# yuguangnudt/VEC_VAD

Hardware: AMD Instinct MI355X
Metric: spatio-temporal cubes/sec (train step) (higher is better)
Workload: dtype f32

## Files before the change

### include/vecvad_hip.h

```cpp
#ifndef VECVAD_HIP_H
#define VECVAD_HIP_H

#include <stddef.h>
#include <stdint.h>

#ifdef __cplusplus
extern "C" {
#endif

typedef void* vv_stream;

enum vv_status {
  VV_OK = 0,
  VV_ERR_BAD_ARG = 1,
  VV_ERR_LAUNCH = 2,
  VV_ERR_UNSUPPORTED = 3
};

enum vv_in_mode {
  VV_IN_PLAIN = 0,
  VV_IN_ACT = 1,
  VV_IN_POOL = 2,
  VV_IN_CAT = 3,
  VV_IN_CUBE = 4,
// ... 113 lines not shown

int vv_bn_finalize(int32_t G, int32_t C, int32_t ntiles, int64_t count, int32_t train, float momentum, float eps,
                   const float* stats, int64_t stats_gstride, const float* gamma, const float* beta,
                   int64_t param_gstride, float* running_mean, float* running_var, int64_t buf_gstride,
                   float* a, float* b, float* mean, float* invstd, int64_t ab_gstride, vv_stream stream);

#define VV_BNBWD_DZ_BF16 1
#define VV_BNBWD_PARTIALS_PER_CUBE 2
#define VV_BNBWD_Y_BF16 8
#define VV_BNBWD_DA_BF16 4
#define VV_BNBWD_PARTIALS_PER_TILE 16
#define VV_BNBWD_PARTIALS_PER_CTILE 32
#define VV_BNBWD_PARTIALS_PER_TTILE 128
#define VV_BNBWD_PARTIALS_PER_TILE44 64
typedef struct vv_bnbwd_params {
  int32_t G, B, H, W, C;
  int32_t flags;
  const float* y; int64_t y_gstride;
  const float* a; const float* b; const float* mean; const float* invstd; int64_t ab_gstride;
  vv_view dA;
  const float* dpool; int64_t dpool_gstride;
  float* dz; int64_t dz_gstride;
  float* partial;
} vv_bnbwd_params;
int vv_bn_bwd_reduce(const vv_bnbwd_params* p, vv_stream stream);
int vv_bn_bwd_nblk(int32_t B, int32_t H, int32_t W, int32_t C);
int vv_bn_bwd_apply(const vv_bnbwd_params* p, const float* gamma, int64_t param_gstride, float* dgamma, float* dbeta,
                    int64_t grad_gstride, float* scratch , vv_stream stream);
#define VV_BNBWD_TAB_ROWS 7
int vv_bn_bwd_sums(const vv_bnbwd_params* p, const float* gamma, int64_t param_gstride, float* dgamma, float* dbeta,
                   int64_t grad_gstride, float* table, int64_t table_gstride, vv_stream stream);

typedef struct vv_outconv_params {
  int32_t G, B, HW, C;
  const float* y; int64_t y_gstride; const float* a; const float* b; int64_t ab_gstride;
  const float* w; const float* bias; int64_t param_gstride;
  const int32_t* oc;
  const float* tgt0; int32_t tgt0_cstride; int32_t pad0;
  const float* tgt1; int32_t tgt1_cstride; int32_t pad1;
  const int32_t* tgt_src;
  const int32_t* tgt_coff;
  float* out4;
  float* score;
  const float* gscale;
  float* dout4;
} vv_outconv_params;
// ... 138 lines not shown
```

### vec_vad_amd/_lib.py

```python
import ctypes as C
import os

import torch

HERE = os.path.dirname(os.path.abspath(__file__))
LIB_PATH = os.environ.get('VV_LIB_PATH') or os.path.join(HERE, 'csrc', 'libvecvad_hip.so')

c_i32, c_i64, c_f32, c_f64, c_vp = C.c_int32, C.c_int64, C.c_float, C.c_double, C.c_void_p

IN_PLAIN, IN_ACT, IN_POOL, IN_CAT, IN_CUBE, IN_BNBWD = 0, 1, 2, 3, 4, 5
BNBWD_TAB_ROWS = 7
CONV3, CONVT_FWD, CONVT_DGRAD = 0, 1, 2
CONV_BF16 = 1
CONV_SRC_BF16 = 2
PACK_BF16 = 4
BNBWD_DZ_BF16 = 1
BNBWD_PARTIALS_PER_CUBE = 2
BNBWD_DA_BF16 = 4
CONV_OUT_BF16 = 8
CONV_ALLSRC_BF16 = 16
CONV_RELU = 32
CONV_NO_GEMM16 = 64
CONV_NO_RING = 128
BNBWD_Y_BF16 = 8
# ... 29 lines not shown
                ('dy', View), ('partial', c_vp), ('partial_gstride', c_i64),
                ('dy_z', View), ('dy_bn', c_vp), ('dy_bn_gstride', c_i64)]


class PackEntry(C.Structure):
    _fields_ = [('src_off', c_i64), ('dst_off', c_i64), ('mode', c_i32), ('K', c_i32), ('KP', c_i32), ('N', c_i32)]


class ReduceEntry(C.Structure):
    _fields_ = [('kind', c_i32), ('Cin', c_i32), ('Cout', c_i32), ('NCO', c_i32), ('nslab', c_i32), ('block_start', c_i32),
                ('part_off', c_i64), ('grad_off', c_i64), ('grad_gstride', c_i64)]


class FoldEntry(C.Structure):
    _fields_ = [('w_off', c_i64), ('b_off', c_i64), ('g_off', c_i64), ('beta_off', c_i64), ('rm_off', c_i64), ('rv_off', c_i64),
                ('cout', c_i32), ('row', c_i32)]


class BnBwdParams(C.Structure):
    _fields_ = [('G', c_i32), ('B', c_i32), ('H', c_i32), ('W', c_i32), ('C', c_i32), ('flags', c_i32),
                ('y', c_vp), ('y_gstride', c_i64),
                ('a', c_vp), ('b', c_vp), ('mean', c_vp), ('invstd', c_vp), ('ab_gstride', c_i64),
                ('dA', View), ('dpool', c_vp), ('dpool_gstride', c_i64),
                ('dz', c_vp), ('dz_gstride', c_i64), ('partial', c_vp)]


class OutconvParams(C.Structure):
    _fields_ = [('G', c_i32), ('B', c_i32), ('HW', c_i32), ('C', c_i32),
                ('y', c_vp), ('y_gstride', c_i64), ('a', c_vp), ('b', c_vp), ('ab_gstride', c_i64),
                ('w', c_vp), ('bias', c_vp), ('param_gstride', c_i64), ('oc', c_vp),
                ('tgt0', c_vp), ('tgt0_cstride', c_i32), ('pad0', c_i32),
                ('tgt1', c_vp), ('tgt1_cstride', c_i32), ('pad1', c_i32),
                ('tgt_src', c_vp), ('tgt_coff', c_vp), ('out4', c_vp), ('score', c_vp), ('gscale', c_vp),
                ('dout4', c_vp)]


class Conv2dParams(C.Structure):
    _fields_ = [('kind', c_i32), ('R', c_i32), ('stride', c_i32), ('B', c_i32), ('H', c_i32), ('W', c_i32),
                ('Cin', c_i32), ('CinP', c_i32), ('Cout', c_i32), ('CoutP', c_i32), ('src', View), ('w', c_vp),
                ('bias', c_vp), ('slope', c_f32), ('pad0', c_i32), ('out', View)]


_SIGS = {
    'vv_conv2d_mfma': (c_i32, [C.POINTER(Conv2dParams), c_vp]),
    'vv_conv2d_wino': (c_i32, [c_vp, c_i32, c_i32, c_i64, c_vp, c_vp, c_f32, c_vp, c_i32, c_i32, c_i32, c_i32, c_i32, c_i32, c_i32, c_vp]),
    'vv_conv2d_splitk_finish': (c_i32, [c_vp, c_i32, c_i64, c_i32, c_i32, c_vp, c_f32, c_vp, c_i32, c_i32, c_vp]),
    'vv_pack_conv2d': (c_i32, [c_vp, c_vp, c_i32, c_i32, c_i32, c_i32, c_i32, c_i32, c_vp]),
# ... 123 lines not shown
```

### vec_vad_amd/bank.py

```python
import ctypes as C
import math
import os
from collections import OrderedDict
from types import SimpleNamespace

import torch

from . import _lib as L

RAW_C, OF_C = 3, 2
HW0 = 32


def _ceil(a, b):
    return (a + b - 1) // b * b


def _pick_ksplit(groups, ntiles, ncu=256, epilogue=1.5, max_wg=1024):
    best, best_cost = 1, None
    for ks in range(1, ntiles + 1):
        if groups * ks > max_wg and ks > 1:
            break
        rounds = -(-groups * ks // ncu)
        cost = rounds * (-(-ntiles // ks) + epilogue)
# ... 158 lines not shown
        def launch_set(name, default, words, names):
            v = os.environ.get(name, default).lower()
            if v.startswith('set:'):
                picked = frozenset(t for t in v[4:].split(',') if t)
                if not picked <= names:
                    raise ValueError('%s=%s: unknown entries %s' % (name, v, sorted(picked - names)))
                return picked
            if v not in words:
                raise ValueError('%s must be one of %s or set:..., got %r' % (name, ' / '.join(words), v))
            return '0' if v == 'off' else v

        self.precision = os.environ.get('VV_PRECISION', 'fp32').lower()
        if self.precision not in ('fp32', 'bf16'):
            raise ValueError("VV_PRECISION / [mi355x] precision must be 'fp32' or 'bf16', got %r" % self.precision)
        if self.nf != 32 and self.precision != 'fp32':
            raise L.VecVadHipError('mixed precision is implemented for features_root = 32 only')
        self.cflag = L.CONV_BF16 if self.precision == 'bf16' else 0
        self.dz16 = switch('VV_BF16_DZ') and bool(self.cflag)
        self.da16 = switch('VV_BF16_DA') and bool(self.cflag)
        self.y16 = switch('VV_BF16_Y') and self.dz16 and self.da16
        self.split_dcat = switch('VV_SPLIT_DCAT') and self.da16
        self.fflag = self.cflag | ((L.CONV_OUT_BF16 | L.CONV_ALLSRC_BF16) if self.y16 else 0)
        self.fuse_outconv = switch('VV_FUSE_OUTCONV')
        wino_env = switch('VV_WINOGRAD')
        self.wino = wino_env and not self.cflag
        self.wino_wgrad = switch('VV_WINOGRAD_WGRAD') and wino_env
        self.wgrad_flag = 256
        w44_words = ('0', 'off', '1', 'dgrad', 'all')
        w44_names = frozenset(['f%d' % i for i in range(nconv)] + ['d%d' % i for i in range(1, nconv)])
        self.w44_mode = launch_set('VV_WINO44', 'dgrad', w44_words, w44_names)
        self._w44_tables = {}
        self._w44_eval_used = set()
        self.w44_eval_mode = launch_set('VV_WINO44_EVAL', '1', w44_words, w44_names)
        self.fuse_bn_sums = switch('VV_FUSE_BN_SUMS')
        self.fuse_bn_sums_t = switch('VV_FUSE_BN_SUMS_T')
        fold = launch_set('VV_FUSE_BN_APPLY', '1', ('0', 'off', '1'), frozenset(str(i) for i in range(nconv)))
        self.fold_bn_apply = frozenset(int(t) for t in fold) if isinstance(fold, frozenset) else \
            frozenset() if fold == '0' else frozenset((0, 2, 4))
        self.group_reduce = switch('VV_GROUP_REDUCE')
        self.eval_fold = switch('VV_EVAL_FOLD') and not self.cflag

        self.params = torch.zeros(G, lay.U, device=d)
        self.bufs = torch.zeros(G, lay.UB, device=d)
        self.gb = [0, lay.p['c4.w'][0], lay.p['c8.w'][0], lay.U]
        self._gb_c = (C.c_int64 * len(self.gb))(*self.gb)
        self.grads = torch.zeros(G * lay.U, device=d)
# ... 218 lines not shown
                    ents[i] = L.PackEntry(lay.p[src][0], off, mode, K, KP, N)
                    mx = max(mx, KP * N)
                self._w44_tables[B] = (torch.frombuffer(bytearray(bytes(ents)), dtype=torch.uint8).to(self.device), len(keys), mx)
        return self._w44_tables[B]

    def _src_for(self, ws, l):
        lay, Ga = self.lay, self.Ga
        abg = lay.cmax
        if l.mode == L.IN_CUBE:
            return (L.IN_PLAIN, L.view(ws.erased, l.cinp, 0, ws.erased.stride(0)), None, None, L.NULL_VIEW, 0, None)
        if l.mode == L.IN_POOL:
            pb = ws.pooled[l.idx]
            return (L.IN_PLAIN, L.view(pb, l.cin, 0, pb.stride(0)), None, None, L.NULL_VIEW, 0, None)
        if l.mode == L.IN_ACT:
            s = lay.convs[l.src]
            y = ws.y[s.idx]
            return (L.IN_ACT, L.view(y, s.cout, 0, y.stride(0)), self._p(ws.ab[0, s.idx]), self._p(ws.ab[1, s.idx]), L.NULL_VIEW, 0, None)
        s = lay.convs[l.skip]
        y, t = ws.y[s.idx], ws.t[l.up]
        return (L.IN_CAT, L.view(y, s.cout, 0, y.stride(0)), self._p(ws.ab[0, s.idx]), self._p(ws.ab[1, s.idx]),
                L.view(t, t.shape[2], 0, t.stride(0)), s.cout, None)

    def _alloc_outconv_bwd(self, ws, B):
        if hasattr(ws, 'gA_last'):
            return
        lib, lay, Ga = self.lib, self.lay, self.Ga
        d = self.device
        f = lambda *shape: torch.empty(*shape, device=d, dtype=torch.float32)
        HWp = HW0 * HW0
        ws.gA_last = f(Ga, B * HWp, self.nf)
        nblk = [lib.vv_bn_bwd_nblk(B, l.H, l.H, l.cout) for l in lay.convs]
        ws.bnpart = f(Ga, max(max(n, lib.vv_wino_ntiles(B, l.H), lib.vv_conv_ntiles(B, l.H, l.H),
                                  lib.vv_conv_ntiles2(B, l.H, l.H, L.CONV3, self.fflag),
                                  lib.vv_convt_dgrad_ntiles(B, l.H, l.H, 0))
                              * 2 * l.cout for n, l in zip(nblk, lay.convs)))
        ws.ocpart = f(Ga, B, 4 * self.nf + 4)

    def backward_plan(self, ws, fused):
        if ws.bwd is None:
            ws.bwd = self._plan_backward(ws, ws.B)
        if not fused:
            return ws.bwd
        if ws.bwdq is None:
            q = _Plan()
            q.keep = ws.bwd.keep
            for c, m in zip(ws.bwd.calls, ws.bwd.meta):
                if c[2] != 'outconv_bwd':
                    q.calls.append(c)
                    q.meta.append(m)
            ws.bwdq = q
        return ws.bwdq

    def _plan_forward(self, ws, B, train, out4=True):
# ... 49 lines not shown
                              L.view(t, co, 0, t.stride(0)), None)
            P.keep.append(cp)
            P.add(lib.vv_conv_mfma, (C.byref(cp),), 'convT%d' % u)

        P.add(lib.vv_cube_erase, (Ga, B * HW0 * HW0, ws.cube.shape[2], lay.convs[0].cinp, ws.cube.data_ptr(),
                                  self._p(self.chmap, g0 * lay.convs[0].cinp), ws.erased.data_ptr(), ws.erased.stride(0),
                                  1 if self.y16 else 0), 'cube_erase')
        for l in lay.convs:
            if l.mode == L.IN_CAT:
                convT(l.up)
            if l.mode == L.IN_POOL:
                s = lay.convs[l.src]
                ys, pb = ws.y[s.idx], ws.pooled[l.idx]
                P.add(lib.vv_pool_act, (Ga, B, l.H, l.H, s.cout, ys.data_ptr(), ys.stride(0), self._p(ws.ab[0, s.idx]),
                                        self._p(ws.ab[1, s.idx]), abg, pb.data_ptr(), pb.stride(0), 1 if self.y16 else 0), 'pool%d' % l.idx)
            conv(l)
        last = lay.convs[-1]
        y = ws.y[last.idx]
        op = L.OutconvParams(Ga, B, HW0 * HW0, self.nf, y.data_ptr(), y.stride(0), self._p(ws.ab[0, last.idx]),
                             self._p(ws.ab[1, last.idx]), abg, pbase + 4 * lay.p['o.w'][0], pbase + 4 * lay.p['o.b'][0], U,
                             self._p(self.oc, g0), ws.cube.data_ptr(), ws.cube.shape[2], 1 if self.y16 else 0, ws.flow.data_ptr(),
                             ws.flow.shape[2], 0, self._p(self.tsrc, g0), self._p(self.tcoff, g0), ws.out4.data_ptr() if out4 else None,
                             ws.score.data_ptr(), ws.gscale.data_ptr() if train else None,
                             ws.dout4.data_ptr() if (train and not (self.fuse_outconv and not out4)) else None)
        P.keep.append(op)
        if train and self.fuse_outconv and not out4:
            P.fused_outconv = True
            P.add(lib.vv_outconv_fwdbwd, (C.byref(op), ws.gA_last.data_ptr(), ws.gA_last.stride(0), ws.ocpart.data_ptr(),
                                          self._p(ws.ab[2, last.idx]), self._p(ws.ab[3, last.idx]), ws.bnpart.data_ptr(),
                                          (1 if self.da16 else 0) | (2 if self.y16 else 0)), 'outconv')
        else:
            P.add(lib.vv_outconv_fwd, (C.byref(op),), 'outconv')
        return P

    def mark_dirty(self):
        self._state_ver += 1

    def prepare_eval(self):
        key = (self._state_ver, self.params._version, self.bufs._version, self.params.data_ptr())
        if self._eval_key == key:
            return
        lib, lay, G = self.lib, self.lay, self.G
        if self.params_eval is None:
            self.params_eval = torch.empty_like(self.params)
            self.packed_eval = torch.zeros_like(self.packed)
        st = self._stream()
        self.params_eval.copy_(self.params)
        L.check(lib.vv_fold_bn(self.fold_table.data_ptr(), len(lay.convs), G, self.params.data_ptr(), lay.U, self.bufs.data_ptr(),
                               lay.UB, 1e-5, self.params_eval.data_ptr(), lay.U, st), 'fold_bn')
        L.check(lib.vv_pack_weights(self.pack_table.data_ptr(), self.pack_n, G, self.params_eval.data_ptr(), lay.U,
                                    self.packed_eval.data_ptr(), lay.UP, self.pack_max, st), 'pack (eval)')
# ... 90 lines not shown

        def dcat_views(m):
            dcat = ws.D[m.idx]
            skipc = lay.convs[m.skip].cout
            if self.split_dcat and 2 * skipc == m.cin and skipc & (skipc - 1) == 0:
                plane = B * m.H * m.H * skipc * 2
                return (L.view(dcat, skipc, 0, dcat.stride(0)), L.view(dcat.data_ptr() + plane, skipc, 0, dcat.stride(0)), skipc)
            return (L.view(dcat, m.cin, 0, dcat.stride(0)), L.View(dcat.data_ptr(), dcat.stride(0), m.cin, skipc), 0)
        ws.DT = [f(Ga, B * H * H, ci) for (_, H, ci, co) in lay.convT]
        ws.dz2 = [f(Ga, B * HWp * nf), f(Ga, B * HWp * nf)]
        ws.dz = ws.dz2[0]
        ws.bnscr = f(Ga, 2 * lay.cmax)
        ws.bscr = f(Ga, (B * HWp + 1023) // 1024 * lay.cmax)
        ws.dstats = f(Ga, max(max(lib.vv_conv_ntiles2(B, l.H, l.H, L.CONV3, self.cflag), lib.vv_conv_ntiles(B, l.H, l.H),
                                  lib.vv_wino_ntiles(B, l.H)) * 2 * l.cin for l in lay.convs if l.mode == L.IN_CAT))

        t_of = {sidx: u for u, (sidx, _, _, _) in enumerate(lay.convT)}
        skip_of = {m.skip: m for m in lay.convs if m.mode == L.IN_CAT}
        pool_of = {m.src: m for m in lay.convs if m.mode == L.IN_POOL}
        act_of = {m.src: m for m in lay.convs if m.mode == L.IN_ACT}

        def dA_for(i):
            if i == last.idx:
                return L.view(ws.gA_last, nf, 0, ws.gA_last.stride(0)), None, 0
            if i in t_of:
                t = ws.DT[t_of[i]]
                return L.view(t, t.shape[2], 0, t.stride(0)), None, 0
            if i in skip_of:
                dp = ws.D[pool_of[i].idx] if i in pool_of else None
                return dcat_views(skip_of[i])[0], dp.data_ptr() if dp is not None else None, dp.stride(0) if dp is not None else 0
            dn = ws.D[i + 1]
            return L.view(dn, lay.convs[i + 1].cin, 0, dn.stride(0)), None, 0

        def wgrad(kind, H, cinp, cout, bf16_flags, wide):
            tiles = ((cinp + 31) // 32) * (cout // 32)
            nt = lib.vv_wgrad_ntiles(kind, B, H, H)
            ks = _pick_ksplit(Ga * tiles, nt, ncu=3 * self.ncu, max_wg=12 * self.ncu) if wide else \
                _pick_ksplit(Ga * tiles, nt, ncu=self.ncu, max_wg=4 * self.ncu)
            w = SimpleNamespace(bf16=False, ks=ks, kw=0)
            ntb, nblk, kw = C.c_int32(), C.c_int32(), C.c_int32()
            if self.cflag and lib.vv_wgrad_bf16_plan(kind | (bf16_flags << 8), B, H, H, cinp, cout,
                                                     C.byref(ntb), C.byref(nblk), C.byref(kw)):
                w = SimpleNamespace(bf16=True, ks=self._ks_bf16(Ga * nblk.value, ntb.value), kw=kw.value)
            w.nslab = w.ks * max(w.kw, 1)
            w.size = tiles * w.nslab * 9 * 1024
            return w
# ... 44 lines not shown
                return
            pending.append((kind, cin, cinp, cout, w, gptr, gstride))
            if not bucket_done:
                return
            ents = (L.ReduceEntry * len(pending))()
            start = 0
            for n, (kind, cin, cinp, cout, w, gptr, gstride) in enumerate(pending):
                ents[n] = L.ReduceEntry(kind, cin, cout, cout // 32, w.nslab, start, w.woff, (gptr - self.grads.data_ptr()) // 4, gstride)
                start += ((cinp + 31) // 32) * (cout // 32) * 36
            tab = torch.frombuffer(bytearray(bytes(ents)), dtype=torch.uint8).to(d)
            P.keep.append(tab)
            P.add(lib.vv_wgrad_reduce_grouped, (tab.data_ptr(), len(pending), start, Ga, ws.wpart.data_ptr(), wpg, self.grads.data_ptr()),
                  label, stream=1, **kw_)
            del pending[:]

        def bn_sums(cp, j):
            yj = ws.y[j]
            cp.bn_z, cp.bn_z_gstride = yj.data_ptr(), yj.stride(0)
            cp.bn_a, cp.bn_b = self._p(ws.ab[0, j]), self._p(ws.ab[1, j])
            cp.bn_mean, cp.bn_invstd = self._p(ws.ab[2, j]), self._p(ws.ab[3, j])
            cp.bn_gstride, cp.bn_partial = abg, ws.bnpart.data_ptr()

        y = ws.y[last.idx]
        P.add(lib.vv_outconv_bwd, (Ga, B, HWp, nf, ws.dout4.data_ptr(), y.data_ptr(), y.stride(0), self._p(ws.ab[0, last.idx]),
                                   self._p(ws.ab[1, last.idx]), abg, pbase + 4 * lay.p['o.w'][0], U, ws.gA_last.data_ptr(),
                                   ws.gA_last.stride(0), ws.ocpart.data_ptr(),
                                   self._p(ws.ab[2, last.idx]), self._p(ws.ab[3, last.idx]), ws.bnpart.data_ptr(),
                                   (1 if self.da16 else 0) | (2 if self.y16 else 0)), 'outconv_bwd')
        assert self._g('o.w')[1] == self._g('o.b')[1]
        P.add(lib.vv_outconv_bwd_reduce, (Ga, nf, B, ws.ocpart.data_ptr(), self._p(self.oc, g0), self._g('o.w')[0],
                                          self._g('o.b')[0], self._g('o.w')[1]), 'outconv_bwd_reduce')

        order = [l.idx for l in reversed(lay.convs)]

        def conv_bwd(l):
            i, r = l.idx, rec[l.idx]
            y = ws.y[i]
            pos = order.index(i)
            dzb = ws.dz2[pos % 2]
            reuse_wait = ('wdone%d' % order[pos - 2],) if pos >= 2 and not r.fold else ()
            bp = L.BnBwdParams(Ga, B, l.H, l.H, l.cout,
                               (L.BNBWD_DZ_BF16 if r.dz16 else 0) | r.partials | (L.BNBWD_DA_BF16 if self.da16 else 0) |
                               (L.BNBWD_Y_BF16 if self.y16 else 0), y.data_ptr(), y.stride(0), self._p(ws.ab[0, i]), self._p(ws.ab[1, i]),
                               self._p(ws.ab[2, i]), self._p(ws.ab[3, i]), abg, r.dA, r.dpool, r.dpg, dzb.data_ptr(), dzb.stride(0),
                               ws.bnpart.data_ptr())
            P.keep.append(bp)
            if not r.partials:
                P.add(lib.vv_bn_bwd_reduce, (C.byref(bp),), 'bn_bwd_reduce%d' % i, wait=reuse_wait)
            if r.fold:
                tab = ws.bntab[i]
                P.add(lib.vv_bn_bwd_sums, (C.byref(bp), pbase + 4 * lay.p['c%d.g' % i][0], U, self._g('c%d.g' % i)[0],
                                           self._g('c%d.beta' % i)[0], self._g('c%d.g' % i)[1], tab.data_ptr(), tab.stride(0)),
                      'bn_bwd_sum%d' % i, record='dy%d' % i)
            else:
                P.add(lib.vv_bn_bwd_apply, (C.byref(bp), pbase + 4 * lay.p['c%d.g' % i][0], U, self._g('c%d.g' % i)[0],
                                            self._g('c%d.beta' % i)[0], self._g('c%d.g' % i)[1], ws.bnscr.data_ptr()), 'bn_bwd_apply%d' % i,
                      record='dy%d' % i, wait=reuse_wait if r.partials else ())
            if i > 0:
                Dl = ws.D[i]
                fn, panel = r.dgrad[:2]
                cp = L.ConvParams(L.CONV3, L.IN_PLAIN, Ga, B, l.H, l.H, l.cout, l.cout, l.cin,
                                  L.View(dzb.data_ptr(), dzb.stride(0), l.cout, 0), None, None, 0, L.NULL_VIEW, 0, r.dflags, None,
                                  kbase + 4 * panel, UP, None, 0, L.view(Dl, l.cin, 0, Dl.stride(0)),
                                  ws.dstats.data_ptr() if l.mode == L.IN_CAT else None)
                if r.fold:
                    cp.in_mode, cp.src0, cp.src1 = L.IN_BNBWD, r.dA, L.view(y, l.cout, 0, y.stride(0))
                    cp.a, cp.ab_gstride = ws.bntab[i].data_ptr(), ws.bntab[i].stride(0)
                if l.mode == L.IN_CAT:
# ... 186 lines not shown
```

### vec_vad_amd/csrc/vv_common.h

```cpp
#pragma once
#include <hip/hip_runtime.h>
#include <stdint.h>
#include <type_traits>
#include "../../include/vecvad_hip.h"

typedef float v16f __attribute__((ext_vector_type(16)));
typedef float v4f __attribute__((ext_vector_type(4)));

#define VV_WG 256

template <int B, int E, typename F>
__device__ __forceinline__ void vv_static_for(F&& f) {
  if constexpr (B < E) {
    f(std::integral_constant<int, B>{});
    vv_static_for<B + 1, E>(f);
  }
}

#define VV_LAUNCH(...)                  \
  do {                                  \
    (void)hipGetLastError();            \
    hipLaunchKernelGGL(__VA_ARGS__);    \
  } while (0)

// ... 37 lines not shown
__device__ __forceinline__ VVBnBwd4 vv_bnbwd_consts(const float* tab, const int C, const int c) {
  VVBnBwd4 k;
  k.a = *reinterpret_cast<const float4*>(tab + c);
  k.b = *reinterpret_cast<const float4*>(tab + C + c);
  k.m = *reinterpret_cast<const float4*>(tab + 2 * C + c);
  k.i = *reinterpret_cast<const float4*>(tab + 3 * C + c);
  k.gk = *reinterpret_cast<const float4*>(tab + 4 * C + c);
  k.c1 = *reinterpret_cast<const float4*>(tab + 5 * C + c);
  k.c2 = *reinterpret_cast<const float4*>(tab + 6 * C + c);
  return k;
}
__device__ __forceinline__ float vv_bnbwd1(float d, const float y, const float a, const float b, const float m, const float i,
                                           const float gk, const float c1, const float c2) {
  const float z = fmaf(a, y, b);
  d = z > 0.f ? d : 0.f;
  const float xh = (y - m) * i;
  return gk * (d - c1 - xh * c2);
}
__device__ __forceinline__ float4 vv_bnbwd4(const float4 d, const float4 y, const VVBnBwd4& k) {
  return make_float4(vv_bnbwd1(d.x, y.x, k.a.x, k.b.x, k.m.x, k.i.x, k.gk.x, k.c1.x, k.c2.x),
                     vv_bnbwd1(d.y, y.y, k.a.y, k.b.y, k.m.y, k.i.y, k.gk.y, k.c1.y, k.c2.y),
                     vv_bnbwd1(d.z, y.z, k.a.z, k.b.z, k.m.z, k.i.z, k.gk.z, k.c1.z, k.c2.z),
                     vv_bnbwd1(d.w, y.w, k.a.w, k.b.w, k.m.w, k.i.w, k.gk.w, k.c1.w, k.c2.w));
}
__device__ __forceinline__ float4 vv_max4(float4 p, float4 q) {
  p.x = fmaxf(p.x, q.x); p.y = fmaxf(p.y, q.y); p.z = fmaxf(p.z, q.z); p.w = fmaxf(p.w, q.w);
  return p;
}

typedef __bf16 v8bf __attribute__((ext_vector_type(8)));
typedef __bf16 v2bf __attribute__((ext_vector_type(2)));
typedef float v2f __attribute__((ext_vector_type(2)));
__device__ __forceinline__ v2f vv_pk_lo_pm_hi(const v2f x, const v2f y) {
  v2f r;
  asm("v_pk_add_f32 %0, %1, %2 op_sel:[0,1] op_sel_hi:[0,1] neg_hi:[0,1]" : "=v"(r) : "v"(x), "v"(y));
  return r;
}

template <int LPP>
__device__ __forceinline__ float vv_group_sum(float d) {
  static_assert(LPP == 8 || LPP == 16, "8 or 16 lanes per group");
  auto dpp = [](const float v, const auto CTRL) -> float {
    return __builtin_bit_cast(float, __builtin_amdgcn_update_dpp(0, __builtin_bit_cast(int, v), decltype(CTRL)::value, 0xF, 0xF, false));
  };
  d += dpp(d, std::integral_constant<int, 0xB1>{});
  d += dpp(d, std::integral_constant<int, 0x4E>{});
// ... 416 lines not shown
```

### vec_vad_amd/csrc/vv_elem.hip

```cpp
#include "vv_common.h"

namespace {

__global__ void __launch_bounds__(VV_WG)
pack_weights_kernel(const vv_pack_entry* __restrict__ table, const float* __restrict__ params,
                    const int64_t params_gstride, float* __restrict__ packed, const int64_t packed_gstride) {
  __shared__ float tile[8 * 32 * 9 + 8];
  const vv_pack_entry e = table[blockIdx.y];
  const int g = blockIdx.z;
  const float* src = params + (int64_t)g * params_gstride + e.src_off;
  float* dst = packed + (int64_t)g * packed_gstride + e.dst_off;
  const bool b16 = (e.mode & 4) != 0;
  const int m = e.mode & 3;
  const bool kmajor = m == 1 || m == 2;
  const bool flip = m == 1;
  const int NB = e.N >> 5, KB = e.KP >> 3;
  const int tid = threadIdx.x;
  for (int blk = blockIdx.x; blk < KB * NB; blk += gridDim.x) {
    const int kb = blk / NB, nb = blk % NB;
    const int k0 = kb * 8, n0 = nb * 32;
    __syncthreads();
    for (int i = tid; i < 8 * 32 * 9; i += VV_WG) {
      int64_t si;
      bool ok;
// ... 72 lines not shown
  double mu, var;
  if (train) {
    double s1 = 0.0, s2 = 0.0;
#pragma unroll
    for (int k = 0; k < VV_NP; ++k) { s1 += sh[0][k][cl]; s2 += sh[1][k][cl]; }
    mu = s1 / count;
    var = s2 / count - mu * mu;
    if (var < 0.0) var = 0.0;
    const double unb = count > 1.0 ? var * count / (count - 1.0) : var;
    *rm = (float)((1.0 - (double)momentum) * (double)*rm + (double)momentum * mu);
    *rv = (float)((1.0 - (double)momentum) * (double)*rv + (double)momentum * unb);
  } else {
    mu = (double)*rm;
    var = (double)*rv;
  }
  const double is = 1.0 / sqrt(var + (double)eps);
  const int64_t o = (int64_t)g * ab_gstride + c;
  a[o] = (float)((double)gm * is);
  b[o] = (float)((double)bt - mu * (double)gm * is);
  mean[o] = (float)mu;
  invstd[o] = (float)is;
}

template <bool POOL, int PASS>
__global__ void __launch_bounds__(VV_WG)
bn_bwd_reduce_kernel(const vv_bnbwd_params p, const int nblk, const int bp, const float* __restrict__ gamma,
                     const int64_t param_gstride, const float* __restrict__ scratch) {
  __shared__ float sh[2][VV_WG * 4];
  const int g = blockIdx.y, blk = blockIdx.x;
  const int C = p.C, Q4 = C >> 2, PL = VV_WG / Q4;
  const int q = threadIdx.x % Q4, pl = threadIdx.x / Q4;
  const int c = q * 4;
  const int64_t M = (int64_t)p.B * p.H * p.W;
  const float* __restrict__ y = p.y + (int64_t)g * p.y_gstride;
  float* __restrict__ dz = p.dz + (int64_t)g * p.dz_gstride;
  const float* __restrict__ dA = p.dA.ptr + (int64_t)g * p.dA.gstride + p.dA.coff;
  const int dcs = p.dA.cstride;
  const bool da16 = (p.flags & VV_BNBWD_DA_BF16) != 0;
  const unsigned short* __restrict__ dAh = reinterpret_cast<const unsigned short*>(p.dA.ptr + (int64_t)g * p.dA.gstride) + p.dA.coff;
  auto ldA = [&](const int64_t pix) -> float4 {
    if (da16) return vv_unpack_bf16x4(*reinterpret_cast<const uint2*>(dAh + pix * dcs + c));
    return *reinterpret_cast<const float4*>(dA + pix * dcs + c);
  };
  const int64_t abo = (int64_t)g * p.ab_gstride + c;
  const float4 a4 = *reinterpret_cast<const float4*>(p.a + abo), b4 = *reinterpret_cast<const float4*>(p.b + abo);
  const float4 m4 = *reinterpret_cast<const float4*>(p.mean + abo), i4 = *reinterpret_cast<const float4*>(p.invstd + abo);
  float4 s1 = make_float4(0, 0, 0, 0), s2 = make_float4(0, 0, 0, 0);
  VVBnBwd4 kc;
  if constexpr (PASS == 1) {
    const float4 gm = *reinterpret_cast<const float4*>(gamma + (int64_t)g * param_gstride + c);
    kc.a = a4; kc.b = b4; kc.m = m4; kc.i = i4;
    kc.gk = make_float4(gm.x * i4.x, gm.y * i4.y, gm.z * i4.z, gm.w * i4.w);
    kc.c1 = *reinterpret_cast<const float4*>(scratch + (int64_t)g * 2 * C + c);
    kc.c2 = *reinterpret_cast<const float4*>(scratch + (int64_t)g * 2 * C + C + c);
  }

  const bool y16 = (p.flags & VV_BNBWD_Y_BF16) != 0;
  auto ldY = [&](const int64_t pix) -> float4 {
    if (y16) return vv_unpack_bf16x4(*reinterpret_cast<const uint2*>(reinterpret_cast<const unsigned short*>(y) + pix * C + c));
    return *reinterpret_cast<const float4*>(y + pix * C + c);
  };
  auto one = [&](const int64_t pix, float4 d, const float4 yv) {
    if constexpr (PASS == 0) {
// ... 337 lines not shown
  const float4 a4 = *reinterpret_cast<const float4*>(a + abo), b4 = *reinterpret_cast<const float4*>(b + abo);
  float4 wv[4];
#pragma unroll
  for (int co = 0; co < 4; ++co) wv[co] = *reinterpret_cast<const float4*>(w + (int64_t)g * param_gstride + co * C + c);
  const float* __restrict__ yg = y + (int64_t)g * y_gstride;
  float* __restrict__ dAg = dA + (int64_t)g * dA_gstride;
  const int64_t MB = (int64_t)B * HW;
  float4 dw[4];
  float db[4] = {0, 0, 0, 0};
#pragma unroll
  for (int co = 0; co < 4; ++co) dw[co] = make_float4(0, 0, 0, 0);
  float4 m4 = make_float4(0, 0, 0, 0), i4 = m4, s1 = m4, s2 = m4;
  if (bnpart) { m4 = *reinterpret_cast<const float4*>(mean + abo); i4 = *reinterpret_cast<const float4*>(invstd + abo); }
  auto ldd = [&](const int i) -> float4 { return *reinterpret_cast<const float4*>(dout4 + ((int64_t)g * MB + (int64_t)cube * HW + i) * 4); };
  auto ldy = [&](const int i) -> float4 {
    const int64_t pix = (int64_t)cube * HW + i;
    return (dA_bf16 & 2) ? vv_unpack_bf16x4(*reinterpret_cast<const uint2*>(reinterpret_cast<const unsigned short*>(yg) + pix * C + c))
                         : *reinterpret_cast<const float4*>(yg + pix * C + c);
  };
  auto body = [&](const int i, const float4 d, const float4 yv) {
    const int64_t pix = (int64_t)cube * HW + i;
    const float4 v = vv_act4(yv, a4, b4);
    const float dd[4] = {d.x, d.y, d.z, d.w};
    float4 o = make_float4(0, 0, 0, 0);
#pragma unroll
    for (int co = 0; co < 4; ++co) {
      o.x = fmaf(dd[co], wv[co].x, o.x); o.y = fmaf(dd[co], wv[co].y, o.y);
      o.z = fmaf(dd[co], wv[co].z, o.z); o.w = fmaf(dd[co], wv[co].w, o.w);
      dw[co].x = fmaf(dd[co], v.x, dw[co].x); dw[co].y = fmaf(dd[co], v.y, dw[co].y);
      dw[co].z = fmaf(dd[co], v.z, dw[co].z); dw[co].w = fmaf(dd[co], v.w, dw[co].w);
      db[co] += dd[co];
    }
    if (dA_bf16 & 1) {
      const uint2 h = vv_pack_bf16x4(o);
      *reinterpret_cast<uint2*>(reinterpret_cast<unsigned short*>(dAg) + pix * C + c) = h;
      o = vv_unpack_bf16x4(h);
    } else {
      *reinterpret_cast<float4*>(dAg + pix * C + c) = o;
    }
    if (bnpart) {
      const float4 gq = make_float4(v.x > 0.f ? o.x : 0.f, v.y > 0.f ? o.y : 0.f, v.z > 0.f ? o.z : 0.f, v.w > 0.f ? o.w : 0.f);
      s1.x += gq.x; s1.y += gq.y; s1.z += gq.z; s1.w += gq.w;
      s2.x = fmaf(gq.x, (yv.x - m4.x) * i4.x, s2.x); s2.y = fmaf(gq.y, (yv.y - m4.y) * i4.y, s2.y);
      s2.z = fmaf(gq.z, (yv.z - m4.z) * i4.z, s2.z); s2.w = fmaf(gq.w, (yv.w - m4.w) * i4.w, s2.w);
    }
  };
  for (int i0 = pg; i0 < HW; i0 += 4 * NPG) {
    float4 d4[4], y4[4];
#pragma unroll
    for (int u = 0; u < 4; ++u)
      if (i0 + u * NPG < HW) { d4[u] = ldd(i0 + u * NPG); y4[u] = ldy(i0 + u * NPG); }
#pragma unroll
    for (int u = 0; u < 4; ++u)
      if (i0 + u * NPG < HW) body(i0 + u * NPG, d4[u], y4[u]);
  }
#pragma unroll
  for (int co = 0; co < 4; ++co) *reinterpret_cast<float4*>(&sh[pg][sub * 16 + co * 4]) = dw[co];
  if (sub == 0) {
#pragma unroll
    for (int co = 0; co < 4; ++co) sh[pg][LPP * 16 + co] = db[co];
// ... 348 lines not shown
    const int64_t pix = (int64_t)cube * p.HW + i;
    const float4 v = vv_act4(yv, a4, b4);
    float o[4];
#pragma unroll
    for (int co = 0; co < 4; ++co) {
      float d = v.x * wv[co].x;
      d = fmaf(v.y, wv[co].y, d); d = fmaf(v.z, wv[co].z, d); d = fmaf(v.w, wv[co].w, d);
      d = vv_group_sum<LPP>(d);
      o[co] = d + bias[co];
    }
    const float tv[4] = {tq.x, tq.y, tq.z, tq.w};
    float e[4] = {0, 0, 0, 0}, dd[4];
#pragma unroll
    for (int co = 0; co < 4; ++co) {
      if (co < oc) e[co] = o[co] - tv[co]; else o[co] = 0.f;
      dd[co] = gs * e[co];
    }
    if (sub == 0) {
#pragma unroll
      for (int co = 0; co < 4; ++co) if (co < oc) sse = fmaf(e[co], e[co], sse);
      if (p.out4) *reinterpret_cast<float4*>(p.out4 + ((int64_t)g * MB + pix) * 4) = make_float4(o[0], o[1], o[2], o[3]);
      if (p.dout4) *reinterpret_cast<float4*>(p.dout4 + ((int64_t)g * MB + pix) * 4) = make_float4(dd[0], dd[1], dd[2], dd[3]);
    }
    float4 q = make_float4(0, 0, 0, 0);
#pragma unroll
    for (int co = 0; co < 4; ++co) {
      q.x = fmaf(dd[co], wb[co].x, q.x); q.y = fmaf(dd[co], wb[co].y, q.y);
      q.z = fmaf(dd[co], wb[co].z, q.z); q.w = fmaf(dd[co], wb[co].w, q.w);
      dw[co].x = fmaf(dd[co], v.x, dw[co].x); dw[co].y = fmaf(dd[co], v.y, dw[co].y);
      dw[co].z = fmaf(dd[co], v.z, dw[co].z); dw[co].w = fmaf(dd[co], v.w, dw[co].w);
      db[co] += dd[co];
    }
    if (flags & 1) {
      const uint2 h = vv_pack_bf16x4(q);
      *reinterpret_cast<uint2*>(reinterpret_cast<unsigned short*>(dAg) + pix * C + c) = h;
      q = vv_unpack_bf16x4(h);
    } else {
      *reinterpret_cast<float4*>(dAg + pix * C + c) = q;
    }
    if (bnpart) {
      const float4 gq = make_float4(v.x > 0.f ? q.x : 0.f, v.y > 0.f ? q.y : 0.f, v.z > 0.f ? q.z : 0.f, v.w > 0.f ? q.w : 0.f);
      s1.x += gq.x; s1.y += gq.y; s1.z += gq.z; s1.w += gq.w;
      s2.x = fmaf(gq.x, (yv.x - m4.x) * i4.x, s2.x); s2.y = fmaf(gq.y, (yv.y - m4.y) * i4.y, s2.y);
      s2.z = fmaf(gq.z, (yv.z - m4.z) * i4.z, s2.z); s2.w = fmaf(gq.w, (yv.w - m4.w) * i4.w, s2.w);
    }
  };
  for (int i0 = pg; i0 < p.HW; i0 += 4 * NPG) {
    float4 yq4[4], tq4[4];
#pragma unroll
    for (int u = 0; u < 4; ++u)
      if (i0 + u * NPG < p.HW) { yq4[u] = ldy(i0 + u * NPG); tq4[u] = ldt(i0 + u * NPG); }
#pragma unroll
    for (int u = 0; u < 4; ++u)
      if (i0 + u * NPG < p.HW) body(i0 + u * NPG, yq4[u], tq4[u]);
  }
#pragma unroll
  for (int off = 32; off >= 1; off >>= 1) sse += __shfl_xor(sse, off);
  if ((tid & 63) == 0) red[tid >> 6] = sse;
#pragma unroll
  for (int co = 0; co < 4; ++co) *reinterpret_cast<float4*>(&sh[pg][sub * 16 + co * 4]) = dw[co];
// ... 336 lines not shown
  return (p->flags & VV_BNBWD_PARTIALS_PER_CUBE) ? p->B
         : (p->flags & VV_BNBWD_PARTIALS_PER_TILE) ? vv_wino_ntiles(p->B, p->H)
         : (p->flags & VV_BNBWD_PARTIALS_PER_TILE44) ? vv_wino44_ntiles(p->B, p->H)
         : (p->flags & VV_BNBWD_PARTIALS_PER_CTILE) ? vv_conv_ntiles(p->B, p->H, p->W)
         : (p->flags & VV_BNBWD_PARTIALS_PER_TTILE) ? vv_convt_dgrad_ntiles(p->B, p->H, p->W, 0) : bn_nblk_of(p);
}

extern "C" int vv_bn_bwd_sums(const vv_bnbwd_params* p, const float* gamma, int64_t param_gstride, float* dgamma, float* dbeta,
                              int64_t grad_gstride, float* table, int64_t table_gstride, vv_stream stream) {
  if (!p || !p->partial || !p->a || !p->b || !p->mean || !p->invstd || !gamma || !dgamma || !dbeta || !table) return VV_ERR_BAD_ARG;
  if (p->dpool || (p->flags & (VV_BNBWD_DZ_BF16 | VV_BNBWD_DA_BF16 | VV_BNBWD_Y_BF16))) return VV_ERR_UNSUPPORTED;
  if (table_gstride < (int64_t)VV_BNBWD_TAB_ROWS * p->C) return VV_ERR_BAD_ARG;
  const int nblk = bn_partial_rows(p);
  if (nblk <= 0) return VV_ERR_BAD_ARG;
  const int64_t M = (int64_t)p->B * p->H * p->W;
  VV_LAUNCH(bn_bwd_sum_kernel, dim3((p->C + 31) / 32, p->G), dim3(32 * VV_NP), 0, (hipStream_t)stream, p->C, nblk, (double)M,
            p->partial, dgamma, dbeta, grad_gstride, nullptr, *p, gamma, param_gstride, table, table_gstride);
  VV_CHECK_LAUNCH();
  return VV_OK;
}

extern "C" int vv_bn_bwd_apply(const vv_bnbwd_params* p, const float* gamma, int64_t param_gstride, float* dgamma,
                               float* dbeta, int64_t grad_gstride, float* scratch, vv_stream stream) {
  if (!p || !p->y || !p->dA.ptr || !p->dz || !p->partial || !gamma || !dgamma || !dbeta || !scratch) return VV_ERR_BAD_ARG;
  const int nblk = bn_partial_rows(p);
  if (nblk <= 0) return VV_ERR_BAD_ARG;
  const int nblk_apply = bn_nblk_of(p);
  const int64_t M = (int64_t)p->B * p->H * p->W;
  VV_LAUNCH(bn_bwd_sum_kernel, dim3((p->C + 31) / 32, p->G), dim3(32 * VV_NP), 0, (hipStream_t)stream, p->C, nblk, (double)M,
            p->partial, dgamma, dbeta, grad_gstride, scratch, *p, nullptr, 0, nullptr, 0);
  VV_CHECK_LAUNCH();
  if (bn_all16(p)) {
    if (p->dpool)
      VV_LAUNCH((bn_bwd16_kernel<true, 1>), dim3(nblk_apply, p->G), dim3(VV_WG), 0, (hipStream_t)stream, *p, nblk_apply, bn_bp_of(p), gamma, param_gstride, scratch);
    else
      VV_LAUNCH((bn_bwd16_kernel<false, 1>), dim3(nblk_apply, p->G), dim3(VV_WG), 0, (hipStream_t)stream, *p, nblk_apply, bn_bp_of(p), gamma, param_gstride, scratch);
  } else if (p->dpool)
    VV_LAUNCH((bn_bwd_reduce_kernel<true, 1>), dim3(nblk_apply, p->G), dim3(VV_WG), 0, (hipStream_t)stream, *p, nblk_apply, bn_bp_of(p), gamma, param_gstride, scratch);
  else
    VV_LAUNCH((bn_bwd_reduce_kernel<false, 1>), dim3(nblk_apply, p->G), dim3(VV_WG), 0, (hipStream_t)stream, *p, nblk_apply, bn_bp_of(p), gamma, param_gstride, scratch);
  VV_CHECK_LAUNCH();
  return VV_OK;
}

extern "C" int vv_outconv_fwd(const vv_outconv_params* p, vv_stream stream) {
  if (!p || !p->y || !p->a || !p->b || !p->w || !p->bias || !p->oc || !p->tgt_src || !p->tgt_coff || !p->score || !p->tgt0)
    return VV_ERR_BAD_ARG;
  if (p->pad0 & 1) return launch_outconv8<0>(*p, nullptr, nullptr, 0, nullptr, nullptr, nullptr, nullptr, true, false, (hipStream_t)stream);
  const int total = p->B * p->G, nper = (total + 7) / 8;
  if (p->C == 32) VV_LAUNCH(outconv_fwd_kernel<32>, dim3(nper * 8), dim3(VV_WG), 0, (hipStream_t)stream, *p, total, nper);
  else if (p->C == 64) VV_LAUNCH(outconv_fwd_kernel<64>, dim3(nper * 8), dim3(VV_WG), 0, (hipStream_t)stream, *p, total, nper);
  else return VV_ERR_UNSUPPORTED;
  VV_CHECK_LAUNCH();
  return VV_OK;
}

extern "C" int vv_outconv_fwdbwd(const vv_outconv_params* p, float* dA, int64_t dA_gstride, float* partial, const float* mean,
                                 const float* invstd, float* bnpart, int32_t flags, vv_stream stream) {
  if (!p || !p->y || !p->a || !p->b || !p->w || !p->bias || !p->oc || !p->tgt_src || !p->tgt_coff || !p->score || !p->tgt0 ||
      !p->gscale || !dA || !partial)
    return VV_ERR_BAD_ARG;
  if (bnpart && (!mean || !invstd)) return VV_ERR_BAD_ARG;
  if (((flags & 2) != 0) != ((p->pad0 & 1) != 0)) return VV_ERR_BAD_ARG;
  if (flags & 2) return launch_outconv8<2>(*p, nullptr, dA, dA_gstride, partial, mean, invstd, bnpart, true, (flags & 1) != 0, (hipStream_t)stream);
  const int total = p->B * p->G, nper = (total + 7) / 8;
  if (p->C == 32) VV_LAUNCH(outconv_fwdbwd_kernel<32>, dim3(nper * 8), dim3(VV_WG), 0, (hipStream_t)stream, *p, dA, dA_gstride, partial, mean, invstd, bnpart, flags, total, nper);
  else if (p->C == 64) VV_LAUNCH(outconv_fwdbwd_kernel<64>, dim3(nper * 8), dim3(VV_WG), 0, (hipStream_t)stream, *p, dA, dA_gstride, partial, mean, invstd, bnpart, flags, total, nper);
  else return VV_ERR_UNSUPPORTED;
  VV_CHECK_LAUNCH();
  return VV_OK;
}

extern "C" int vv_outconv_bwd_nblk(int32_t B, int32_t HW) { (void)HW; return B; }

extern "C" int vv_outconv_bwd(int32_t G, int32_t B, int32_t HW, int32_t C, const float* dout4, const float* y,
                              int64_t y_gstride, const float* a, const float* b, int64_t ab_gstride, const float* w,
                              int64_t param_gstride, float* dA, int64_t dA_gstride, float* partial,
                              const float* mean, const float* invstd, float* bnpart, int32_t dA_bf16, vv_stream stream) {
  if (!dout4 || !y || !a || !b || !w || !dA || !partial) return VV_ERR_BAD_ARG;
  if (bnpart && (!mean || !invstd)) return VV_ERR_BAD_ARG;
  if (dA_bf16 & 2) {
    vv_outconv_params p = {};
    p.G = G; p.B = B; p.HW = HW; p.C = C;
    p.y = y; p.y_gstride = y_gstride; p.a = a; p.b = b; p.ab_gstride = ab_gstride;
    p.w = w; p.param_gstride = param_gstride;
    return launch_outconv8<1>(p, dout4, dA, dA_gstride, partial, mean, invstd, bnpart, true, (dA_bf16 & 1) != 0, (hipStream_t)stream);
  }
  if (C == 32)
    VV_LAUNCH(outconv_bwd_kernel<32>, dim3(B, G), dim3(VV_WG), 0, (hipStream_t)stream, B, HW, C, dout4, y, y_gstride,
              a, b, ab_gstride, w, param_gstride, dA, dA_gstride, partial, mean, invstd, bnpart, dA_bf16);
  else if (C == 64)
    VV_LAUNCH(outconv_bwd_kernel<64>, dim3(B, G), dim3(VV_WG), 0, (hipStream_t)stream, B, HW, C, dout4, y, y_gstride,
              a, b, ab_gstride, w, param_gstride, dA, dA_gstride, partial, mean, invstd, bnpart, dA_bf16);
  else return VV_ERR_UNSUPPORTED;
  VV_CHECK_LAUNCH();
  return VV_OK;
}

extern "C" int vv_outconv_bwd_reduce(int32_t G, int32_t C, int32_t nblk, const float* partial, const int32_t* oc,
                                     float* dW, float* db, int64_t grad_gstride, vv_stream stream) {
  if (!partial || !oc || !dW || !db) return VV_ERR_BAD_ARG;
  if (C == 32) VV_LAUNCH(outconv_bwd_reduce_kernel<32>, dim3(G), dim3(1024), 0, (hipStream_t)stream, C, nblk, partial, oc, dW, db, grad_gstride);
// ... 222 lines not shown
```

Baseline: 29080.

## Recompute output-conv dA in BN backward apply instead of storing it

In fp32 mode by default, the outconv backward no longer writes the full-size dA tensor for the last layer. The BN backward apply kernel instead rebuilds dA on the fly from the 4-channel dout4 and the outconv weights. This removes a large write and read-back of B*HW*nf floats in exchange for a few extra FMAs per element. The dout4 buffer is now always written in the fused path, which adds a small store.

```diff
diff --git a/include/vecvad_hip.h b/include/vecvad_hip.h
--- a/include/vecvad_hip.h
+++ b/include/vecvad_hip.h
@@ -159,6 +159,7 @@
   const float* dpool; int64_t dpool_gstride;
   float* dz; int64_t dz_gstride;
   float* partial;
+  const float* oc_dout4; const float* oc_w; int64_t oc_w_gstride;
 } vv_bnbwd_params;
 int vv_bn_bwd_reduce(const vv_bnbwd_params* p, vv_stream stream);
 int vv_bn_bwd_nblk(int32_t B, int32_t H, int32_t W, int32_t C);
diff --git a/vec_vad_amd/_lib.py b/vec_vad_amd/_lib.py
--- a/vec_vad_amd/_lib.py
+++ b/vec_vad_amd/_lib.py
@@ -75,7 +75,8 @@
                 ('y', c_vp), ('y_gstride', c_i64),
                 ('a', c_vp), ('b', c_vp), ('mean', c_vp), ('invstd', c_vp), ('ab_gstride', c_i64),
                 ('dA', View), ('dpool', c_vp), ('dpool_gstride', c_i64),
-                ('dz', c_vp), ('dz_gstride', c_i64), ('partial', c_vp)]
+                ('dz', c_vp), ('dz_gstride', c_i64), ('partial', c_vp),
+                ('oc_dout4', c_vp), ('oc_w', c_vp), ('oc_w_gstride', c_i64)]
 
 
 class OutconvParams(C.Structure):
diff --git a/vec_vad_amd/bank.py b/vec_vad_amd/bank.py
--- a/vec_vad_amd/bank.py
+++ b/vec_vad_amd/bank.py
@@ -204,6 +204,10 @@
         self.split_dcat = switch('VV_SPLIT_DCAT') and self.da16
         self.fflag = self.cflag | ((L.CONV_OUT_BF16 | L.CONV_ALLSRC_BF16) if self.y16 else 0)
         self.fuse_outconv = switch('VV_FUSE_OUTCONV')
+        oda = os.environ.get('VV_OUTCONV_DA', 'load').lower()
+        if oda not in ('load', 'store'):
+            raise ValueError("VV_OUTCONV_DA must be 'load' or 'store', got %r" % oda)
+        self.outconv_da_load = oda == 'load' and not self.cflag
         wino_env = switch('VV_WINOGRAD')
         self.wino = wino_env and not self.cflag
         self.wino_wgrad = switch('VV_WINOGRAD_WGRAD') and wino_env
@@ -468,13 +472,14 @@
                 L.view(t, t.shape[2], 0, t.stride(0)), s.cout, None)
 
     def _alloc_outconv_bwd(self, ws, B):
-        if hasattr(ws, 'gA_last'):
+        if hasattr(ws, 'ocpart'):
             return
         lib, lay, Ga = self.lib, self.lay, self.Ga
         d = self.device
         f = lambda *shape: torch.empty(*shape, device=d, dtype=torch.float32)
         HWp = HW0 * HW0
-        ws.gA_last = f(Ga, B * HWp, self.nf)
+        if not self.outconv_da_load:
+            ws.gA_last = f(Ga, B * HWp, self.nf)
         nblk = [lib.vv_bn_bwd_nblk(B, l.H, l.H, l.cout) for l in lay.convs]
         ws.bnpart = f(Ga, max(max(n, lib.vv_wino_ntiles(B, l.H), lib.vv_conv_ntiles(B, l.H, l.H),
                                   lib.vv_conv_ntiles2(B, l.H, l.H, L.CONV3, self.fflag),
@@ -570,11 +575,12 @@
                              self._p(self.oc, g0), ws.cube.data_ptr(), ws.cube.shape[2], 1 if self.y16 else 0, ws.flow.data_ptr(),
                              ws.flow.shape[2], 0, self._p(self.tsrc, g0), self._p(self.tcoff, g0), ws.out4.data_ptr() if out4 else None,
                              ws.score.data_ptr(), ws.gscale.data_ptr() if train else None,
-                             ws.dout4.data_ptr() if (train and not (self.fuse_outconv and not out4)) else None)
+                             ws.dout4.data_ptr() if (train and (self.outconv_da_load or not (self.fuse_outconv and not out4))) else None)
         P.keep.append(op)
         if train and self.fuse_outconv and not out4:
             P.fused_outconv = True
-            P.add(lib.vv_outconv_fwdbwd, (C.byref(op), ws.gA_last.data_ptr(), ws.gA_last.stride(0), ws.ocpart.data_ptr(),
+            gA = (None, 0) if self.outconv_da_load else (ws.gA_last.data_ptr(), ws.gA_last.stride(0))
+            P.add(lib.vv_outconv_fwdbwd, (C.byref(op), gA[0], gA[1], ws.ocpart.data_ptr(),
                                           self._p(ws.ab[2, last.idx]), self._p(ws.ab[3, last.idx]), ws.bnpart.data_ptr(),
                                           (1 if self.da16 else 0) | (2 if self.y16 else 0)), 'outconv')
         else:
@@ -711,6 +717,8 @@
 
         def dA_for(i):
             if i == last.idx:
+                if self.outconv_da_load:
+                    return L.NULL_VIEW, None, 0
                 return L.view(ws.gA_last, nf, 0, ws.gA_last.stride(0)), None, 0
             if i in t_of:
                 t = ws.DT[t_of[i]]
@@ -801,9 +809,9 @@
             cp.bn_gstride, cp.bn_partial = abg, ws.bnpart.data_ptr()
 
         y = ws.y[last.idx]
+        gA = (None, 0) if self.outconv_da_load else (ws.gA_last.data_ptr(), ws.gA_last.stride(0))
         P.add(lib.vv_outconv_bwd, (Ga, B, HWp, nf, ws.dout4.data_ptr(), y.data_ptr(), y.stride(0), self._p(ws.ab[0, last.idx]),
-                                   self._p(ws.ab[1, last.idx]), abg, pbase + 4 * lay.p['o.w'][0], U, ws.gA_last.data_ptr(),
-                                   ws.gA_last.stride(0), ws.ocpart.data_ptr(),
+                                   self._p(ws.ab[1, last.idx]), abg, pbase + 4 * lay.p['o.w'][0], U, gA[0], gA[1], ws.ocpart.data_ptr(),
                                    self._p(ws.ab[2, last.idx]), self._p(ws.ab[3, last.idx]), ws.bnpart.data_ptr(),
                                    (1 if self.da16 else 0) | (2 if self.y16 else 0)), 'outconv_bwd')
         assert self._g('o.w')[1] == self._g('o.b')[1]
@@ -823,6 +831,8 @@
                                (L.BNBWD_Y_BF16 if self.y16 else 0), y.data_ptr(), y.stride(0), self._p(ws.ab[0, i]), self._p(ws.ab[1, i]),
                                self._p(ws.ab[2, i]), self._p(ws.ab[3, i]), abg, r.dA, r.dpool, r.dpg, dzb.data_ptr(), dzb.stride(0),
                                ws.bnpart.data_ptr())
+            if i == last.idx and self.outconv_da_load:
+                bp.oc_dout4, bp.oc_w, bp.oc_w_gstride = ws.dout4.data_ptr(), pbase + 4 * lay.p['o.w'][0], U
             P.keep.append(bp)
             if not r.partials:
                 P.add(lib.vv_bn_bwd_reduce, (C.byref(bp),), 'bn_bwd_reduce%d' % i, wait=reuse_wait)
diff --git a/vec_vad_amd/csrc/vv_common.h b/vec_vad_amd/csrc/vv_common.h
--- a/vec_vad_amd/csrc/vv_common.h
+++ b/vec_vad_amd/csrc/vv_common.h
@@ -83,6 +83,16 @@
                      vv_bnbwd1(d.y, y.y, k.a.y, k.b.y, k.m.y, k.i.y, k.gk.y, k.c1.y, k.c2.y),
                      vv_bnbwd1(d.z, y.z, k.a.z, k.b.z, k.m.z, k.i.z, k.gk.z, k.c1.z, k.c2.z),
                      vv_bnbwd1(d.w, y.w, k.a.w, k.b.w, k.m.w, k.i.w, k.gk.w, k.c1.w, k.c2.w));
+}
+__device__ __forceinline__ float4 vv_outconv_dA4(const float4 d, const float4 (&w)[4]) {
+  const float dd[4] = {d.x, d.y, d.z, d.w};
+  float4 o = make_float4(0, 0, 0, 0);
+#pragma unroll
+  for (int co = 0; co < 4; ++co) {
+    o.x = fmaf(dd[co], w[co].x, o.x); o.y = fmaf(dd[co], w[co].y, o.y);
+    o.z = fmaf(dd[co], w[co].z, o.z); o.w = fmaf(dd[co], w[co].w, o.w);
+  }
+  return o;
 }
 __device__ __forceinline__ float4 vv_max4(float4 p, float4 q) {
   p.x = fmaxf(p.x, q.x); p.y = fmaxf(p.y, q.y); p.z = fmaxf(p.z, q.z); p.w = fmaxf(p.w, q.w);
diff --git a/vec_vad_amd/csrc/vv_elem.hip b/vec_vad_amd/csrc/vv_elem.hip
--- a/vec_vad_amd/csrc/vv_elem.hip
+++ b/vec_vad_amd/csrc/vv_elem.hip
@@ -118,7 +118,7 @@
   invstd[o] = (float)is;
 }
 
-template <bool POOL, int PASS>
+template <bool POOL, int PASS, bool OC = false>
 __global__ void __launch_bounds__(VV_WG)
 bn_bwd_reduce_kernel(const vv_bnbwd_params p, const int nblk, const int bp, const float* __restrict__ gamma,
                      const int64_t param_gstride, const float* __restrict__ scratch) {
@@ -134,7 +134,13 @@
   const int dcs = p.dA.cstride;
   const bool da16 = (p.flags & VV_BNBWD_DA_BF16) != 0;
   const unsigned short* __restrict__ dAh = reinterpret_cast<const unsigned short*>(p.dA.ptr + (int64_t)g * p.dA.gstride) + p.dA.coff;
+  float4 wo[4];
+  if constexpr (OC) {
+#pragma unroll
+    for (int co = 0; co < 4; ++co) wo[co] = *reinterpret_cast<const float4*>(p.oc_w + (int64_t)g * p.oc_w_gstride + co * C + c);
+  }
   auto ldA = [&](const int64_t pix) -> float4 {
+    if constexpr (OC) return vv_outconv_dA4(*reinterpret_cast<const float4*>(p.oc_dout4 + ((int64_t)g * M + pix) * 4), wo);
     if (da16) return vv_unpack_bf16x4(*reinterpret_cast<const uint2*>(dAh + pix * dcs + c));
     return *reinterpret_cast<const float4*>(dA + pix * dcs + c);
   };
@@ -518,11 +524,9 @@
     const int64_t pix = (int64_t)cube * HW + i;
     const float4 v = vv_act4(yv, a4, b4);
     const float dd[4] = {d.x, d.y, d.z, d.w};
-    float4 o = make_float4(0, 0, 0, 0);
+    float4 o = vv_outconv_dA4(d, wv);
 #pragma unroll
     for (int co = 0; co < 4; ++co) {
-      o.x = fmaf(dd[co], wv[co].x, o.x); o.y = fmaf(dd[co], wv[co].y, o.y);
-      o.z = fmaf(dd[co], wv[co].z, o.z); o.w = fmaf(dd[co], wv[co].w, o.w);
       dw[co].x = fmaf(dd[co], v.x, dw[co].x); dw[co].y = fmaf(dd[co], v.y, dw[co].y);
       dw[co].z = fmaf(dd[co], v.z, dw[co].z); dw[co].w = fmaf(dd[co], v.w, dw[co].w);
       db[co] += dd[co];
@@ -531,7 +535,7 @@
       const uint2 h = vv_pack_bf16x4(o);
       *reinterpret_cast<uint2*>(reinterpret_cast<unsigned short*>(dAg) + pix * C + c) = h;
       o = vv_unpack_bf16x4(h);
-    } else {
+    } else if (dA) {
       *reinterpret_cast<float4*>(dAg + pix * C + c) = o;
     }
     if (bnpart) {
@@ -926,11 +930,9 @@
       if (p.out4) *reinterpret_cast<float4*>(p.out4 + ((int64_t)g * MB + pix) * 4) = make_float4(o[0], o[1], o[2], o[3]);
       if (p.dout4) *reinterpret_cast<float4*>(p.dout4 + ((int64_t)g * MB + pix) * 4) = make_float4(dd[0], dd[1], dd[2], dd[3]);
     }
-    float4 q = make_float4(0, 0, 0, 0);
+    float4 q = vv_outconv_dA4(make_float4(dd[0], dd[1], dd[2], dd[3]), wb);
 #pragma unroll
     for (int co = 0; co < 4; ++co) {
-      q.x = fmaf(dd[co], wb[co].x, q.x); q.y = fmaf(dd[co], wb[co].y, q.y);
-      q.z = fmaf(dd[co], wb[co].z, q.z); q.w = fmaf(dd[co], wb[co].w, q.w);
       dw[co].x = fmaf(dd[co], v.x, dw[co].x); dw[co].y = fmaf(dd[co], v.y, dw[co].y);
       dw[co].z = fmaf(dd[co], v.z, dw[co].z); dw[co].w = fmaf(dd[co], v.w, dw[co].w);
       db[co] += dd[co];
@@ -939,7 +941,7 @@
       const uint2 h = vv_pack_bf16x4(q);
       *reinterpret_cast<uint2*>(reinterpret_cast<unsigned short*>(dAg) + pix * C + c) = h;
       q = vv_unpack_bf16x4(h);
-    } else {
+    } else if (dA) {
       *reinterpret_cast<float4*>(dAg + pix * C + c) = q;
     }
     if (bnpart) {
@@ -1322,7 +1324,10 @@
 
 extern "C" int vv_bn_bwd_apply(const vv_bnbwd_params* p, const float* gamma, int64_t param_gstride, float* dgamma,
                                float* dbeta, int64_t grad_gstride, float* scratch, vv_stream stream) {
-  if (!p || !p->y || !p->dA.ptr || !p->dz || !p->partial || !gamma || !dgamma || !dbeta || !scratch) return VV_ERR_BAD_ARG;
+  if (!p || !p->y || !(p->dA.ptr || p->oc_dout4) || !p->dz || !p->partial || !gamma || !dgamma || !dbeta || !scratch) return VV_ERR_BAD_ARG;
+  const bool oc = p->oc_dout4 != nullptr;
+  if (oc && (!p->oc_w || p->dA.ptr || p->dpool || (p->flags & (VV_BNBWD_DZ_BF16 | VV_BNBWD_DA_BF16 | VV_BNBWD_Y_BF16)))) return VV_ERR_BAD_ARG;
+  if (oc && (p->C % 4 || p->C > 1024 || VV_WG % (p->C / 4))) return VV_ERR_UNSUPPORTED;
   const int nblk = bn_partial_rows(p);
   if (nblk <= 0) return VV_ERR_BAD_ARG;
   const int nblk_apply = bn_nblk_of(p);
@@ -1337,6 +1342,8 @@
       VV_LAUNCH((bn_bwd16_kernel<false, 1>), dim3(nblk_apply, p->G), dim3(VV_WG), 0, (hipStream_t)stream, *p, nblk_apply, bn_bp_of(p), gamma, param_gstride, scratch);
   } else if (p->dpool)
     VV_LAUNCH((bn_bwd_reduce_kernel<true, 1>), dim3(nblk_apply, p->G), dim3(VV_WG), 0, (hipStream_t)stream, *p, nblk_apply, bn_bp_of(p), gamma, param_gstride, scratch);
+  else if (oc)
+    VV_LAUNCH((bn_bwd_reduce_kernel<false, 1, true>), dim3(nblk_apply, p->G), dim3(VV_WG), 0, (hipStream_t)stream, *p, nblk_apply, bn_bp_of(p), gamma, param_gstride, scratch);
   else
     VV_LAUNCH((bn_bwd_reduce_kernel<false, 1>), dim3(nblk_apply, p->G), dim3(VV_WG), 0, (hipStream_t)stream, *p, nblk_apply, bn_bp_of(p), gamma, param_gstride, scratch);
   VV_CHECK_LAUNCH();
@@ -1358,8 +1365,9 @@
 extern "C" int vv_outconv_fwdbwd(const vv_outconv_params* p, float* dA, int64_t dA_gstride, float* partial, const float* mean,
                                  const float* invstd, float* bnpart, int32_t flags, vv_stream stream) {
   if (!p || !p->y || !p->a || !p->b || !p->w || !p->bias || !p->oc || !p->tgt_src || !p->tgt_coff || !p->score || !p->tgt0 ||
-      !p->gscale || !dA || !partial)
+      !p->gscale || !partial)
     return VV_ERR_BAD_ARG;
+  if (!dA && (!p->dout4 || (flags & 3))) return VV_ERR_BAD_ARG;
   if (bnpart && (!mean || !invstd)) return VV_ERR_BAD_ARG;
   if (((flags & 2) != 0) != ((p->pad0 & 1) != 0)) return VV_ERR_BAD_ARG;
   if (flags & 2) return launch_outconv8<2>(*p, nullptr, dA, dA_gstride, partial, mean, invstd, bnpart, true, (flags & 1) != 0, (hipStream_t)stream);
@@ -1377,7 +1385,8 @@
                               int64_t y_gstride, const float* a, const float* b, int64_t ab_gstride, const float* w,
                               int64_t param_gstride, float* dA, int64_t dA_gstride, float* partial,
                               const float* mean, const float* invstd, float* bnpart, int32_t dA_bf16, vv_stream stream) {
-  if (!dout4 || !y || !a || !b || !w || !dA || !partial) return VV_ERR_BAD_ARG;
+  if (!dout4 || !y || !a || !b || !w || !partial) return VV_ERR_BAD_ARG;
+  if (!dA && (dA_bf16 & 3)) return VV_ERR_BAD_ARG;
   if (bnpart && (!mean || !invstd)) return VV_ERR_BAD_ARG;
   if (dA_bf16 & 2) {
     vv_outconv_params p = {};
```

After: 29250, median of 6. About the same (+0.6%).
